# omuses/hqp

Measured on AMD Instinct MI355X. Metric: KKT factor+solve/sec (fp64), higher is better.
Workload: dtype f64; 1 GPU; C4 = BASELINE configs[3], the metric's 10^6-variable DOCP: multistage LQ optimal control QP, K=200 stages, nx=5000 states, nu=50 controls -> n=1015000 me=1005000 m=20000, dense fx/fu handed over as blocks, x_0 fixed, box bounds on u; plugin LQDOCP (STAGED engine), one system per GPU; stages=200, nx=5000, nu=50, n=1015000, me=1005000, m=20000, plugin=LQDOCP, kkt_dim_full=2040000

## Files before the change

### hqp_amd/csrc/staged.hip.h

```cpp
#pragma once
#include <hip/hip_runtime.h>

#include <algorithm>

#include "staged_plan.hpp"
#include "sk_table.hpp"

namespace stg {

using kktdev::double4_t;
using kktdev::mfma_f64;

typedef double double2_t __attribute__((ext_vector_type(2)));

struct StripTab {
  int nranks;
  int cut[17];
  int ld[17];
  long long off[17];
};
struct RectTab {
  int nranks;
  int cut[17];
  struct Block {
    long long off[2];
    int rsplit;
    int pad;
  } blk[16 * 16];
};
static __device__ __forceinline__ int strip_of(const int *cut, int nranks, int j) {
  int p = 0;
  while (p + 1 < nranks && cut[p + 1] <= j) p++;
  return p;
}

struct GemmArgs {
  const double *A;
  long long lda;
  const double *B;
  long long ldb;
  const double *Cin;
  long long ldcin;
  double *C;
  long long ldc;
  int M, N, K;
  double alpha, beta;
  int lower;
  int mirror;
  const int *tile_map;
  const double *zeros;
  const RectTab *rects;
  const StripTab *bstrips;
  unsigned long long *stamps;
};

static const int GEMM_BK = 16;

static inline long long gemm_tiles(int M, int N, int b, int lower) {
  const long long tm = (M + b - 1) / b, tn = (N + b - 1) / b;
  return lower ? tn * (tn + 1) / 2 + (tm > tn ? (tm - tn) * tn : 0) : tm * tn;
}
static inline size_t gemm_lds_bytes(int bm, int bn, int nbuf = 2) { return sizeof(double) * nbuf * GEMM_BK * (size_t)(bm + 16 + bn + 16); }

static inline bool gemm_big_tiles(int M, int N, int lower, int K = 0) {
  const long long t = gemm_tiles(M, N, 128, lower);
  return t >= 384 || (!lower && t >= 160 && t <= 256 && K >= 256 * GEMM_BK);
}

static inline bool gemm_use_split(int M, int N, int K, int lower, int grid);
__device__ __forceinline__ int xcd_swizzle(int bid, int nwg) {
  const int q = nwg >> 3, r = nwg & 7, x = bid & 7;
  return x * q + (x < r ? x : r) + (bid >> 3);
}

template <int BM, int BN, int WGM = 2, int WGN = 2>
struct GemmTile {
  static constexpr int BK = GEMM_BK;
  static constexpr int NW = WGM * WGN, NT = 64 * NW;
  static constexpr int LDA = BM + 16, LDB = BN + 16;
  static constexpr int WM = BM / WGM, WN = BN / WGN, TM = WM / 16, TN = WN / 16;
  static constexpr int LA = BK * BM / 2 / 256, LB = BK * BN / 2 / 256;
  static constexpr int RA = 256 / (BM / 2), RB = 256 / (BN / 2);

  static __device__ __forceinline__ void tile_of(const GemmArgs &g, int t, int &tm, int &tn) {
    if (g.tile_map && BM == 128) {
      const int e = g.tile_map[t];
      tm = e >> 16, tn = e & 0xffff;
    } else if (g.lower) {
      const int tcols = (g.N + BN - 1) / BN, tri = tcols * (tcols + 1) / 2;
      if (t < tri) {
        tm = (int)((sqrtf(8.0f * (float)t + 1.0f) - 1.0f) * 0.5f);
        while ((tm + 1) * (tm + 2) / 2 <= t) tm++;
        while (tm * (tm + 1) / 2 > t) tm--;
        tn = t - tm * (tm + 1) / 2;
      } else {
        tm = tcols + (t - tri) / tcols;
        tn = (t - tri) % tcols;
      }
    } else {
      const int tiles_n = (g.N + BN - 1) / BN, tiles_m = (g.M + BM - 1) / BM;
      constexpr int GM = 8;
      const int grp = t / (GM * tiles_n), first = grp * GM;
      const int rows = min(GM, tiles_m - first);
      const int in = t - grp * GM * tiles_n;
      tm = first + in % rows;
      tn = in / rows;
    }
  }

  static __device__ __forceinline__ void accumulate(const GemmArgs &g, int i0, int j0, int s0, int s1,
                                                    double4_t (&acc)[TM][TN], double *As, double *Bs) {
    static_assert(NT == 256, "the register-staged loop is written for 256 threads");
    const int tid = threadIdx.x, lane = tid & 63, wave = tid >> 6;
    const int wm = wave / WGN, wn = wave % WGN;
    const int lr = lane & 15, lk = lane >> 4;
    const int ca = 2 * (tid % (BM / 2)), ra = tid / (BM / 2);
    const int cb = 2 * (tid % (BN / 2)), rb = tid / (BN / 2);
    const long long acol = (i0 + ca < g.lda) ? i0 + ca : 0;
    const double *Bp = g.B;
    long long ldb = g.ldb;
    int jb = j0;
    if (g.bstrips) {
      const int q = strip_of(g.bstrips->cut, g.bstrips->nranks, j0);
      Bp = g.B + g.bstrips->off[q], ldb = g.bstrips->ld[q], jb = j0 - g.bstrips->cut[q];
    }
    const long long bcol = (jb + cb < ldb) ? jb + cb : 0;
    constexpr int D = (BM * BN <= 64 * 64) ? 4 : 1;
    double2_t sa[D][LA], sb[D][LB];
    const int last = s1 - 1;
    auto gload = [&](double2_t(&xa)[LA], double2_t(&xb)[LB], int slab) {
      const int k0 = (slab < last ? slab : last) * BK;
#pragma unroll
      for (int p = 0; p < LA; p++) {
        const int k = k0 + ra + p * RA, kc = k < g.K ? k : g.K - 1;
        xa[p] = *(const double2_t *)(g.A + (long long)kc * g.lda + acol);
      }
#pragma unroll
      for (int p = 0; p < LB; p++) {
        const int k = k0 + rb + p * RB, kc = k < g.K ? k : g.K - 1;
        xb[p] = *(const double2_t *)(Bp + (long long)kc * ldb + bcol);
      }
    };
    auto lstore = [&](int buf, const double2_t(&xa)[LA], const double2_t(&xb)[LB], int slab) {
      const int k0 = (slab < last ? slab : last) * BK;
#pragma unroll
      for (int p = 0; p < LA; p++) {
        double2_t v = xa[p];
        if (k0 + ra + p * RA >= g.K) v = (double2_t){0.0, 0.0};
        *(double2_t *)(As + (buf * BK + ra + p * RA) * LDA + ca) = v;
      }
#pragma unroll
      for (int p = 0; p < LB; p++) {
        double2_t v = xb[p];
        if (k0 + rb + p * RB >= g.K) v = (double2_t){0.0, 0.0};
        *(double2_t *)(Bs + (buf * BK + rb + p * RB) * LDB + cb) = v;
      }
    };
    auto multiply = [&](int buf) {
      const double *Ab = As + buf * BK * LDA + wm * WM + lr;
      const double *Bb = Bs + buf * BK * LDB + wn * WN + lr;
#pragma unroll
      for (int ks = 0; ks < BK / 4; ks++) {
        double af[TM], bf[TN];
#pragma unroll
        for (int x = 0; x < TM; x++) af[x] = Ab[(ks * 4 + lk) * LDA + 16 * x];
#pragma unroll
        for (int y = 0; y < TN; y++) bf[y] = Bb[(ks * 4 + lk) * LDB + 16 * y];
#pragma unroll
        for (int x = 0; x < TM; x++)
#pragma unroll
          for (int y = 0; y < TN; y++) acc[x][y] = mfma_f64(af[x], bf[y], acc[x][y]);
      }
    };
    if (s1 <= s0) return;
#pragma unroll
    for (int d = 0; d < D; d++) gload(sa[d], sb[d], s0 + d);
    lstore(0, sa[0], sb[0], s0);
    __syncthreads();
    int s = s0;
    for (; s + D <= s1; s += D) {
#pragma unroll
      for (int d = 0; d < D; d++) {
        const int buf = d & 1;
        gload(sa[d], sb[d], s + d + D);
        multiply(D == 1 ? ((s - s0) & 1) : buf);
        lstore(D == 1 ? (((s - s0) & 1) ^ 1) : (buf ^ 1), sa[(d + 1) % D], sb[(d + 1) % D], s + d + 1);
        __syncthreads();
      }
    }
#pragma unroll
    for (int d = 0; d < D - 1; d++) {
      if (s + d < s1) {
        multiply((D == 1 ? (s + d - s0) : d) & 1);
        if (s + d + 1 < s1) lstore(((D == 1 ? (s + d - s0) : d) & 1) ^ 1, sa[(d + 1) % D], sb[(d + 1) % D], s + d + 1);
        __syncthreads();
      }
    }
  }

  static __device__ __forceinline__ void glds16(const double *src, double *lds_row) {
    __builtin_amdgcn_global_load_lds((const __attribute__((address_space(1))) void *)src,
                                     (__attribute__((address_space(3))) void *)lds_row, 16, 0, 0);
  }
  template <bool MASKED>
  static __device__ __forceinline__ void slabs_dma(const GemmArgs &g, const double *pa, const double *pb, const double *zr, int wave,
                                                   int wm, int wn, int lr, int lk, int s0, int s1, unsigned mask,
                                                   double4_t (&acc)[TM][TN], double *As, double *Bs) {
    constexpr int RPW = BK / NW;
    auto dma = [&](int buf, int k0, int p) {
      const int r = wave + NW * (p % RPW), k = k0 + r;
      if (p < RPW)
        glds16(k < g.K ? pa + (long long)k * g.lda : zr, As + (buf * BK + r) * LDA);
      else
        glds16(k < g.K ? pb + (long long)k * g.ldb : zr, Bs + (buf * BK + r) * LDB);
    };
    if (s1 > s0) {
#pragma unroll
      for (int p = 0; p < 2 * RPW; p++) dma(0, s0 * BK, p);
    }
    __syncthreads();
    constexpr int GAP = TM * TN / (2 * RPW);
    for (int s = s0; s < s1; s++) {
      const int buf = (s - s0) & 1;
      const int knext = s + 1 < s1 ? (s + 1) * BK : g.K;
      const double *Ab = As + buf * BK * LDA + wm * WM + lr;
      const double *Bb = Bs + buf * BK * LDB + wn * WN + lr;
#pragma unroll
      for (int ks = 0; ks < BK / 4; ks++) {
        double af[TM], bf[TN];
#pragma unroll
        for (int x = 0; x < TM; x++) af[x] = Ab[(ks * 4 + lk) * LDA + 16 * x];
#pragma unroll
        for (int y = 0; y < TN; y++) bf[y] = Bb[(ks * 4 + lk) * LDB + 16 * y];
#pragma unroll
        for (int x = 0; x < TM; x++)
#pragma unroll
          for (int y = 0; y < TN; y++) {
            if (!MASKED || ((mask >> (x * TN + y)) & 1u)) acc[x][y] = mfma_f64(af[x], bf[y], acc[x][y]);
            if (ks == 0 && (x * TN + y) % GAP == GAP - 1) dma(buf ^ 1, knext, (x * TN + y) / GAP);
          }
      }
      __syncthreads();
    }
  }
  template <bool MASKED>
  static __device__ __forceinline__ void slabs_dma3(const GemmArgs &g, const double *pa, const double *pb, const double *zr, int wave,
                                                    int wm, int wn, int lr, int lk, int s0, int s1, unsigned mask,
                                                    double4_t (&acc)[TM][TN], double *As, double *Bs) {
    constexpr int RPW = BK / NW;
    static_assert(2 * RPW == 4 || 2 * RPW == 8, "the counted waits below are written for 4 or 8 pieces per wave and slab");
    auto dma = [&](int buf, int k0, int p) {
      const int r = wave + NW * (p % RPW), k = k0 + r;
      if (p < RPW)
        glds16(k < g.K ? pa + (long long)k * g.lda : zr, As + (buf * BK + r) * LDA);
      else
        glds16(k < g.K ? pb + (long long)k * g.ldb : zr, Bs + (buf * BK + r) * LDB);
    };
    auto wait_all_but_newest_slab = [&]() {
      if constexpr (2 * RPW == 4)
        asm volatile("s_waitcnt vmcnt(4) lgkmcnt(0)\n\ts_barrier" ::: "memory");
      else
        asm volatile("s_waitcnt vmcnt(8) lgkmcnt(0)\n\ts_barrier" ::: "memory");
    };
#pragma unroll
    for (int p = 0; p < 2 * RPW; p++) dma(0, s1 > s0 ? s0 * BK : g.K, p);
#pragma unroll
    for (int p = 0; p < 2 * RPW; p++) dma(1, s0 + 1 < s1 ? (s0 + 1) * BK : g.K, p);
    wait_all_but_newest_slab();
    constexpr int GAP = TM * TN / (2 * RPW);
    int buf = 0;
    for (int s = s0; s < s1; s++) {
      const int bnext = buf >= 1 ? buf - 1 : 2;
      const int knext = s + 2 < s1 ? (s + 2) * BK : g.K;
      const double *Ab = As + buf * BK * LDA + wm * WM + lr;
      const double *Bb = Bs + buf * BK * LDB + wn * WN + lr;
#pragma unroll
      for (int ks = 0; ks < BK / 4; ks++) {
        double af[TM], bf[TN];
#pragma unroll
        for (int x = 0; x < TM; x++) af[x] = Ab[(ks * 4 + lk) * LDA + 16 * x];
#pragma unroll
        for (int y = 0; y < TN; y++) bf[y] = Bb[(ks * 4 + lk) * LDB + 16 * y];
#pragma unroll
        for (int x = 0; x < TM; x++)
#pragma unroll
          for (int y = 0; y < TN; y++) {
            if (!MASKED || ((mask >> (x * TN + y)) & 1u)) acc[x][y] = mfma_f64(af[x], bf[y], acc[x][y]);
            if (ks == 0 && (x * TN + y) % GAP == GAP - 1) dma(bnext, knext, (x * TN + y) / GAP);
          }
      }
      wait_all_but_newest_slab();
      buf = buf == 2 ? 0 : buf + 1;
    }
    asm volatile("s_waitcnt vmcnt(0)" ::: "memory");
    __syncthreads();
  }
  static __device__ __forceinline__ void accumulate_dma(const GemmArgs &g, int i0, int j0, int s0, int s1,
                                                        double4_t (&acc)[TM][TN], double *As, double *Bs, bool skip_upper = false, int nbuf = 2) {
    static_assert(BM == 128 && BN == 128, "one k-row of a panel must be one 1-KiB wave-instruction");
    static_assert((BK / NW) * NW == BK && TM * TN >= 2 * (BK / NW) && TM * TN <= 32,
                  "pieces are issued behind the multiplications of the first k-step");
    const int tid = threadIdx.x, lane = tid & 63, wave = __builtin_amdgcn_readfirstlane(tid >> 6);
    const int wm = wave / WGN, wn = wave % WGN;
    const int lr = lane & 15, lk = lane >> 4;
    GemmArgs gl = g;
    int jb = j0;
    if (g.bstrips) {
      const int q = strip_of(g.bstrips->cut, g.bstrips->nranks, j0);
      gl.B = g.B + g.bstrips->off[q], gl.ldb = g.bstrips->ld[q], jb = j0 - g.bstrips->cut[q];
    }
    const double *pa = g.A + ((i0 + 2 * lane < g.lda) ? i0 + 2 * lane : 0);
    const double *pb = gl.B + ((jb + 2 * lane < gl.ldb) ? jb + 2 * lane : 0);
    const double *zr = g.zeros + 2 * lane;
    unsigned mask = 0;
#pragma unroll
    for (int x = 0; x < TM; x++)
#pragma unroll
      for (int y = 0; y < TN; y++) {
        const int rb = wm * TM + x, cb = wn * TN + y;
        const bool want = i0 + 16 * rb < g.M && j0 + 16 * cb < g.N && !(skip_upper && cb > rb);
        mask |= (want ? 1u : 0u) << (x * TN + y);
      }
    mask = __builtin_amdgcn_readfirstlane(mask);
    const bool all = mask == (TM * TN == 32 ? 0xffffffffu : (1u << (TM * TN)) - 1u);
    if (nbuf == 3) {
      if (all)
        slabs_dma3<false>(gl, pa, pb, zr, wave, wm, wn, lr, lk, s0, s1, mask, acc, As, Bs);
      else
        slabs_dma3<true>(gl, pa, pb, zr, wave, wm, wn, lr, lk, s0, s1, mask, acc, As, Bs);
    } else if (all)
      slabs_dma<false>(gl, pa, pb, zr, wave, wm, wn, lr, lk, s0, s1, mask, acc, As, Bs);
    else
      slabs_dma<true>(gl, pa, pb, zr, wave, wm, wn, lr, lk, s0, s1, mask, acc, As, Bs);
  }

  static __device__ __forceinline__ void epilogue(const GemmArgs &g, int tm, int tn, const double4_t (&acc)[TM][TN], double *lds) {
    const int tid = threadIdx.x, lane = tid & 63, wave = tid >> 6;
    const int wm = wave / WGN, wn = wave % WGN;
    const int lr = lane & 15, lk = lane >> 4;
    const int i0 = tm * BM, j0 = tn * BN;
    const bool diag = g.lower && tm == tn;
    const double *cin = g.Cin;
    long long ldcin = g.ldcin;
    if (g.rects && g.beta != 0.0) {
      const RectTab &R = *g.rects;
      const int a = strip_of(R.cut, R.nranks, i0), b = strip_of(R.cut, R.nranks, j0);
      const RectTab::Block &blk = R.blk[a * 16 + b];
      const int t = i0 >= blk.rsplit ? 1 : 0, r0 = t ? blk.rsplit : R.cut[a], c0 = R.cut[b];
      ldcin = R.cut[b + 1] - c0;
      cin = g.Cin + blk.off[t] - ((long long)r0 * ldcin + c0);
    }
    constexpr int HC = BN < 64 ? BN : 64, LDT = BM + 2;
    const bool via_lds = g.mirror && !diag && lds != nullptr;
    double4_t val[TM][TN];
#pragma unroll
    for (int x = 0; x < TM; x++)
#pragma unroll
      for (int y = 0; y < TN; y++)
#pragma unroll
        for (int rg = 0; rg < 4; rg++) {
          const int i = i0 + wm * WM + 16 * x + lk + 4 * rg, j = j0 + wn * WN + 16 * y + lr;
          double v = 0.0;
          if (i < g.M && j < g.N && !(diag && i < j)) {
            v = g.alpha * acc[x][y][rg];
            if (g.beta != 0.0) v += g.beta * cin[(long long)i * ldcin + j];
            g.C[(long long)i * g.ldc + j] = v;
            if (g.mirror && i != j && !via_lds) g.C[(long long)j * g.ldc + i] = v;
          }
          val[x][y][rg] = v;
        }
    if (via_lds) {
#pragma unroll
      for (int h = 0; h < BN / HC; h++) {
        if ((wn * WN) / HC == h) {
#pragma unroll
          for (int x = 0; x < TM; x++)
#pragma unroll
            for (int y = 0; y < TN; y++)
#pragma unroll
              for (int rg = 0; rg < 4; rg++)
                lds[(wn * WN - h * HC + 16 * y + lr) * LDT + wm * WM + 16 * x + lk + 4 * rg] = val[x][y][rg];
        }
        __syncthreads();
        for (int jj = wave; jj < HC; jj += NW) {
          const int j = j0 + h * HC + jj;
          if (j >= g.N) break;
          for (int ii = 2 * lane; ii < BM; ii += 128) {
            const int i = i0 + ii;
            double *dst = g.C + (long long)j * g.ldc + i;
            if (i + 1 < g.M && (((size_t)dst) & 15) == 0)
              *(double2_t *)dst = *(const double2_t *)(lds + jj * LDT + ii);
            else {
              if (i < g.M) dst[0] = lds[jj * LDT + ii];
              if (i + 1 < g.M) dst[1] = lds[jj * LDT + ii + 1];
            }
          }
        }
        __syncthreads();
      }
    }
  }
};

constexpr int gemm_waves_per_simd(int nw, int nbuf) { return nbuf == 3 ? nw / 4 : nw / 2; }
template <int BM, int BN, bool DMA = false, int WGM = 2, int WGN = 2, int NBUF = 2>
__global__ void __launch_bounds__(64 * WGM * WGN, gemm_waves_per_simd(WGM * WGN, NBUF)) k_dgemm_tn(GemmArgs g) {
  using T = GemmTile<BM, BN, WGM, WGN>;
  extern __shared__ __attribute__((aligned(16))) double lds[];
  double *As = lds, *Bs = lds + NBUF * T::BK * ((DMA && BM == 64) ? 64 : T::LDA);
  int tm, tn;
  const unsigned long long t0 = g.stamps ? __builtin_amdgcn_s_memrealtime() : 0;
  T::tile_of(g, xcd_swizzle(blockIdx.x, gridDim.x), tm, tn);
  double4_t acc[T::TM][T::TN];
#pragma unroll
  for (int x = 0; x < T::TM; x++)
#pragma unroll
    for (int y = 0; y < T::TN; y++) acc[x][y] = (double4_t){0.0, 0.0, 0.0, 0.0};
  if constexpr (DMA)
    T::accumulate_dma(g, tm * BM, tn * BN, 0, (g.K + T::BK - 1) / T::BK, acc, As, Bs, g.lower && tm == tn, NBUF);
  else
    T::accumulate(g, tm * BM, tn * BN, 0, (g.K + T::BK - 1) / T::BK, acc, As, Bs);
  const unsigned long long t2 = g.stamps ? __builtin_amdgcn_s_memrealtime() : 0;
  T::epilogue(g, tm, tn, acc, lds);
  if (g.stamps && threadIdx.x == 0) {
    asm volatile("s_waitcnt vmcnt(0)" ::: "memory");
    unsigned xcc;
    asm volatile("s_getreg_b32 %0, hwreg(HW_REG_XCC_ID)" : "=s"(xcc));
    g.stamps[4 * blockIdx.x + 0] = t0, g.stamps[4 * blockIdx.x + 1] = (unsigned long long)(xcc & 15);
    g.stamps[4 * blockIdx.x + 2] = t2, g.stamps[4 * blockIdx.x + 3] = __builtin_amdgcn_s_memrealtime();
  }
}

template <int BM, int BN>
__global__ void __launch_bounds__(256) k_dgemm_tn_ks(GemmArgs g, double *__restrict__ part, int nsplit) {
  using T = GemmTile<BM, BN, 2, 2>;
  extern __shared__ __attribute__((aligned(16))) double lds[];
  double *As = lds, *Bs = lds + 2 * T::BK * T::LDA;
  int tm, tn;
  T::tile_of(g, blockIdx.x, tm, tn);
  const int nslab = (g.K + T::BK - 1) / T::BK, L = (nslab + nsplit - 1) / nsplit;
  const int s0 = min(nslab, (int)blockIdx.y * L), s1 = min(nslab, s0 + L);
  double4_t acc[T::TM][T::TN];
#pragma unroll
  for (int x = 0; x < T::TM; x++)
#pragma unroll
    for (int y = 0; y < T::TN; y++) acc[x][y] = (double4_t){0.0, 0.0, 0.0, 0.0};
  T::accumulate(g, tm * BM, tn * BN, s0, s1, acc, As, Bs);
  const int lane = threadIdx.x & 63, wave = threadIdx.x >> 6, wm = wave / 2, wn = wave % 2, lr = lane & 15, lk = lane >> 4;
  double *out = part + (long long)blockIdx.y * g.M * g.N;
#pragma unroll
  for (int x = 0; x < T::TM; x++)
#pragma unroll
    for (int y = 0; y < T::TN; y++)
#pragma unroll
      for (int rg = 0; rg < 4; rg++) {
        const int i = tm * BM + wm * T::WM + 16 * x + lk + 4 * rg, j = tn * BN + wn * T::WN + 16 * y + lr;
        if (i < g.M && j < g.N) out[(long long)i * g.N + j] = acc[x][y][rg];
      }
}
__global__ void k_dgemm_ks_finish(GemmArgs g, const double *__restrict__ part, int nsplit) {
  const long long e = (long long)blockIdx.x * blockDim.x + threadIdx.x, tot = (long long)g.M * g.N;
  if (e >= tot) return;
  double s = 0.0;
  for (int y = 0; y < nsplit; y++) s += part[(long long)y * tot + e];
  const int i = (int)(e / g.N), j = (int)(e % g.N);
  double v = g.alpha * s;
  if (g.beta != 0.0) v += g.beta * g.Cin[(long long)i * g.ldcin + j];
  g.C[(long long)i * g.ldc + j] = v;
}

struct SplitPlan {
  double *ws;
  unsigned *cnt;
  int dp_rounds;
  int whole;
  int nphase;
  int begin[3], count[3], split[3];
  int frac, per, ntiles;
  const SkUnit *table;
  int stride;
};

static inline SplitPlan gemm_split_plan(long long tiles, long long nslab, int grid) {
  SplitPlan sp{};
  const long long smax = std::max<long long>(1, std::min<long long>(16, nslab / 16));
  sp.dp_rounds = (int)(tiles / grid);
  long long R = tiles - (long long)sp.dp_rounds * grid, begin = (long long)sp.dp_rounds * grid;
  sp.whole = (int)begin;
  while (R > 0 && sp.nphase < 2) {
    long long s = std::min<long long>(smax, grid / R), r = R;
    if (s <= 1) {
      s = 1;
      if (sp.nphase == 0 && smax >= 2 && R > grid / 2 && grid % 2 == 0) s = 2, r = grid / 2;
    }
    sp.begin[sp.nphase] = (int)begin, sp.count[sp.nphase] = (int)r, sp.split[sp.nphase] = (int)s;
    sp.nphase++, begin += r, R -= r;
  }
  return sp;
}
static inline SplitPlan gemm_split_plan_frac(long long tiles, long long nslab, int grid) {
  SplitPlan sp{};
  sp.frac = 1, sp.ntiles = (int)tiles;
  sp.per = (int)((tiles * nslab + grid - 1) / grid);
  return sp;
}
static inline long long gemm_split_plan_pieces(const SplitPlan &sp) {
  long long n = 0;
  for (int q = 0; q < sp.nphase; q++) n += (long long)sp.count[q] * sp.split[q];
  return n;
}
static inline long long gemm_split_plan_depth(const SplitPlan &sp, long long nslab) {
  long long d = (long long)sp.dp_rounds * nslab;
  for (int q = 0; q < sp.nphase; q++) d += (nslab + sp.split[q] - 1) / sp.split[q];
  return d;
}
static inline bool gemm_use_split(int M, int N, int K, int lower, int grid) {
  if (grid <= 0 || (long long)M * N < 256LL * 256) return false;
  const long long tiles = gemm_tiles(M, N, 128, lower);
  const long long nslab = (K + GEMM_BK - 1) / GEMM_BK;
  if (nslab < 32) return false;
  if (tiles % grid == 0 || tiles >= 16LL * grid) return false;
  if (tiles > grid * 5 / 8) return true;
  return false;
}
static inline bool gemm_use_frac(int M, int N, int K, int lower, int grid) {
  if (grid <= 0) return false;
  const long long tiles = gemm_tiles(M, N, 128, lower), nslab = (K + GEMM_BK - 1) / GEMM_BK;
  return nslab >= 64 && tiles * 16 >= grid * 5LL && tiles * 8 <= grid * 5LL;
}
template <bool DMA, int WGM = 2, int WGN = 2, int NBUF = 2, int BM = 128, int BN = 128>
__global__ void __launch_bounds__(64 * WGM * WGN, NBUF == 3 ? WGM * WGN / 4 : WGM * WGN / 2) k_dgemm_tn_sk(GemmArgs g, SplitPlan sk) {
  using T = GemmTile<BM, BN, WGM, WGN>;
  extern __shared__ __attribute__((aligned(16))) double lds[];
  double *As = lds, *Bs = lds + NBUF * T::BK * T::LDA;
  unsigned *s_old = (unsigned *)(lds + NBUF * T::BK * (T::LDA + T::LDB));
  const int G = gridDim.x, v = xcd_swizzle(blockIdx.x, G);
  const int nslab = (g.K + T::BK - 1) / T::BK;
  constexpr int SLOT = BM * BN;
  unsigned long long *stamp = g.stamps ? g.stamps + 32 * (long long)blockIdx.x : nullptr;
  if (stamp && threadIdx.x == 0) stamp[0] = __builtin_amdgcn_s_memrealtime();
  if (sk.table) {
    auto unit = [&](const SkUnit u, int r) {
      const int t = u.tile, s0 = u.s0, s1 = u.s1, pieces = u.pieces, j = u.j;
      int tm, tn;
      T::tile_of(g, t, tm, tn);
      double4_t acc[T::TM][T::TN];
#pragma unroll
      for (int x = 0; x < T::TM; x++)
#pragma unroll
        for (int y = 0; y < T::TN; y++) acc[x][y] = (double4_t){0.0, 0.0, 0.0, 0.0};
      if constexpr (DMA)
        T::accumulate_dma(g, tm * BM, tn * BN, s0, s1, acc, As, Bs, g.lower && tm == tn, NBUF);
      else
        T::accumulate(g, tm * BM, tn * BN, s0, s1, acc, As, Bs);
      bool finish = true;
      if (stamp && threadIdx.x == 0 && r < 10) stamp[1 + 3 * r] = __builtin_amdgcn_s_memrealtime();
      if (pieces > 1) {
        double *mine = sk.ws + (long long)(u.slot0 + j) * SLOT;
#pragma unroll
        for (int x = 0; x < T::TM; x++)
#pragma unroll
          for (int y = 0; y < T::TN; y++)
#pragma unroll
            for (int rg = 0; rg < 4; rg++) mine[((x * T::TN + y) * 4 + rg) * T::NT + threadIdx.x] = acc[x][y][rg];
        asm volatile("s_waitcnt vmcnt(0)" ::: "memory");
        __syncthreads();
        if (threadIdx.x == 0) {
          __builtin_amdgcn_fence(__ATOMIC_RELEASE, "agent");
          asm volatile("s_waitcnt vmcnt(0)" ::: "memory");
          *s_old = __hip_atomic_fetch_add(sk.cnt + t, 1u, __ATOMIC_RELAXED, __HIP_MEMORY_SCOPE_AGENT);
        }
        __syncthreads();
        finish = *s_old == (unsigned)(pieces - 1);
        if (finish) {
          if (threadIdx.x == 0) {
            sk.cnt[t] = 0;
            __builtin_amdgcn_fence(__ATOMIC_ACQUIRE, "agent");
            asm volatile("s_waitcnt vmcnt(0)" ::: "memory");
          }
          __syncthreads();
#pragma unroll
          for (int x = 0; x < T::TM; x++)
#pragma unroll
            for (int y = 0; y < T::TN; y++) acc[x][y] = (double4_t){0.0, 0.0, 0.0, 0.0};
          for (int jj = 0; jj < pieces; jj++) {
            const double *theirs = sk.ws + (long long)(u.slot0 + jj) * SLOT;
#pragma unroll
            for (int x = 0; x < T::TM; x++)
#pragma unroll
              for (int y = 0; y < T::TN; y++)
#pragma unroll
                for (int rg = 0; rg < 4; rg++) acc[x][y][rg] += theirs[((x * T::TN + y) * 4 + rg) * T::NT + threadIdx.x];
          }
        }
        __syncthreads();
      }
      if (stamp && threadIdx.x == 0 && r < 10) stamp[2 + 3 * r] = __builtin_amdgcn_s_memrealtime();
      if (finish) T::epilogue(g, tm, tn, acc, lds);
      if (stamp && threadIdx.x == 0 && r < 10) {
        asm volatile("s_waitcnt vmcnt(0)" ::: "memory");
        stamp[3 + 3 * r] = __builtin_amdgcn_s_memrealtime();
      }
      __syncthreads();
    };
    const SkUnit *tab = sk.table + (long long)blockIdx.x * sk.stride;
    for (int r = 0; r < sk.stride; r++) {
      const SkUnit u = tab[r];
      if (u.tile < 0) break;
      unit(u, r);
    }
    return;
  }
  if (sk.frac) {
    const int U = sk.ntiles * nslab, per = sk.per;
    const int lo = min(U, v * per), hi = min(U, lo + per), t_first = lo / nslab;
    for (int x = lo; x < hi;) {
      const int t = x / nslab, s0 = x - t * nslab, s1 = min(nslab, s0 + (hi - x));
      const int w_first = (t * nslab) / per, w_last = ((t + 1) * nslab - 1) / per, pieces = w_last - w_first + 1;
      int tm, tn;
      T::tile_of(g, t, tm, tn);
      double4_t acc[T::TM][T::TN];
#pragma unroll
      for (int xx = 0; xx < T::TM; xx++)
#pragma unroll
        for (int y = 0; y < T::TN; y++) acc[xx][y] = (double4_t){0.0, 0.0, 0.0, 0.0};
      if constexpr (DMA)
        T::accumulate_dma(g, tm * BM, tn * BN, s0, s1, acc, As, Bs, g.lower && tm == tn, NBUF);
      else
        T::accumulate(g, tm * BM, tn * BN, s0, s1, acc, As, Bs);
      bool finish = true;
      if (pieces > 1) {
        double *mine = sk.ws + (long long)(2 * v + (t == t_first ? 0 : 1)) * SLOT;
#pragma unroll
        for (int xx = 0; xx < T::TM; xx++)
#pragma unroll
          for (int y = 0; y < T::TN; y++)
#pragma unroll
            for (int rg = 0; rg < 4; rg++) mine[((xx * T::TN + y) * 4 + rg) * T::NT + threadIdx.x] = acc[xx][y][rg];
        asm volatile("s_waitcnt vmcnt(0)" ::: "memory");
        __syncthreads();
        if (threadIdx.x == 0) {
          __builtin_amdgcn_fence(__ATOMIC_RELEASE, "agent");
          asm volatile("s_waitcnt vmcnt(0)" ::: "memory");
          *s_old = __hip_atomic_fetch_add(sk.cnt + t, 1u, __ATOMIC_RELAXED, __HIP_MEMORY_SCOPE_AGENT);
        }
        __syncthreads();
        finish = *s_old == (unsigned)(pieces - 1);
        if (finish) {
          if (threadIdx.x == 0) {
            sk.cnt[t] = 0;
            __builtin_amdgcn_fence(__ATOMIC_ACQUIRE, "agent");
            asm volatile("s_waitcnt vmcnt(0)" ::: "memory");
          }
          __syncthreads();
#pragma unroll
          for (int xx = 0; xx < T::TM; xx++)
#pragma unroll
            for (int y = 0; y < T::TN; y++) acc[xx][y] = (double4_t){0.0, 0.0, 0.0, 0.0};
          for (int w = w_first; w <= w_last; w++) {
            const double *theirs = sk.ws + (long long)(2 * w + (t == (w * per) / nslab ? 0 : 1)) * SLOT;
#pragma unroll
            for (int xx = 0; xx < T::TM; xx++)
#pragma unroll
              for (int y = 0; y < T::TN; y++)
#pragma unroll
                for (int rg = 0; rg < 4; rg++) acc[xx][y][rg] += theirs[((xx * T::TN + y) * 4 + rg) * T::NT + threadIdx.x];
          }
        }
        __syncthreads();
      }
      if (finish) T::epilogue(g, tm, tn, acc, lds);
      __syncthreads();
      x += s1 - s0;
    }
    return;
  }
  const int n_whole = sk.whole;
  int n_units = n_whole;
  for (int q = 0; q < sk.nphase; q++) n_units += sk.count[q] * sk.split[q];
  int r = 0;
  for (int u = v; u < n_units; r++) {
    int q = -1;
    int t = u, s0 = 0, s1 = nslab, cnt = G, pieces = 1, ti = 0, pbase = 0;
    if (u >= n_whole) {
      int rel = u - n_whole;
      q = 0;
      while (q + 1 < sk.nphase && rel >= sk.count[q] * sk.split[q]) rel -= sk.count[q] * sk.split[q], pbase += sk.count[q] * sk.split[q], q++;
      cnt = sk.count[q], pieces = sk.split[q];
      ti = rel % cnt;
      const int L = (nslab + pieces - 1) / pieces, j = rel / cnt;
      t = sk.begin[q] + ti, s0 = min(nslab, j * L), s1 = min(nslab, s0 + L);
    }
    const int u_now = u;
    {
      int nu = n_units;
      if (u + G < n_whole)
        nu = u + G;
      else {
        int base = n_whole, qq = 0;
        if (u >= n_whole) base += pbase + cnt * pieces, qq = q + 1;
        for (; qq < sk.nphase && nu == n_units; qq++) {
          if (v < sk.count[qq] * sk.split[qq]) nu = base + v;
          base += sk.count[qq] * sk.split[qq];
        }
      }
      if (threadIdx.x == 0) s_old[1] = (unsigned)nu;
    }
    int tm, tn;
    T::tile_of(g, t, tm, tn);
    double4_t acc[T::TM][T::TN];
#pragma unroll
    for (int x = 0; x < T::TM; x++)
#pragma unroll
      for (int y = 0; y < T::TN; y++) acc[x][y] = (double4_t){0.0, 0.0, 0.0, 0.0};
    if constexpr (DMA)
      T::accumulate_dma(g, tm * BM, tn * BN, s0, s1, acc, As, Bs, g.lower && tm == tn, NBUF);
    else
      T::accumulate(g, tm * BM, tn * BN, s0, s1, acc, As, Bs);
    bool finish = true;
    if (stamp && threadIdx.x == 0 && r < 5) stamp[1 + 3 * r] = __builtin_amdgcn_s_memrealtime();
    if (pieces > 1) {
      double *mine = sk.ws + (long long)(u_now - n_whole) * SLOT;
#pragma unroll
      for (int x = 0; x < T::TM; x++)
#pragma unroll
        for (int y = 0; y < T::TN; y++)
#pragma unroll
          for (int rg = 0; rg < 4; rg++) mine[((x * T::TN + y) * 4 + rg) * T::NT + threadIdx.x] = acc[x][y][rg];
      asm volatile("s_waitcnt vmcnt(0)" ::: "memory");
      __syncthreads();
      if (threadIdx.x == 0) {
        __builtin_amdgcn_fence(__ATOMIC_RELEASE, "agent");
        asm volatile("s_waitcnt vmcnt(0)" ::: "memory");
        *s_old = __hip_atomic_fetch_add(sk.cnt + t, 1u, __ATOMIC_RELAXED, __HIP_MEMORY_SCOPE_AGENT);
      }
      __syncthreads();
      finish = *s_old == (unsigned)(pieces - 1);
      if (finish) {
        if (threadIdx.x == 0) {
          sk.cnt[t] = 0;
          __builtin_amdgcn_fence(__ATOMIC_ACQUIRE, "agent");
          asm volatile("s_waitcnt vmcnt(0)" ::: "memory");
        }
        __syncthreads();
#pragma unroll
        for (int x = 0; x < T::TM; x++)
#pragma unroll
          for (int y = 0; y < T::TN; y++) acc[x][y] = (double4_t){0.0, 0.0, 0.0, 0.0};
        for (int jj = 0; jj < pieces; jj++) {
          const double *theirs = sk.ws + (long long)(pbase + jj * cnt + ti) * SLOT;
#pragma unroll
          for (int x = 0; x < T::TM; x++)
#pragma unroll
            for (int y = 0; y < T::TN; y++)
#pragma unroll
              for (int rg = 0; rg < 4; rg++) acc[x][y][rg] += theirs[((x * T::TN + y) * 4 + rg) * T::NT + threadIdx.x];
        }
      }
      __syncthreads();
    }
    if (stamp && threadIdx.x == 0 && r < 5) stamp[2 + 3 * r] = __builtin_amdgcn_s_memrealtime();
    if (finish) T::epilogue(g, tm, tn, acc, lds);
    if (stamp && threadIdx.x == 0 && r < 5) {
      asm volatile("s_waitcnt vmcnt(0)" ::: "memory");
      stamp[3 + 3 * r] = __builtin_amdgcn_s_memrealtime();
    }
    __syncthreads();
    u = (int)s_old[1];
    __syncthreads();
  }
}
static inline size_t gemm_sk_lds_bytes(int nbuf = 2) { return gemm_lds_bytes(128, 128, nbuf) + 16; }

enum { GEMM_REG4 = 0, GEMM_DMA4 = 1, GEMM_DMA8 = 2, GEMM_DMA8X3 = 3 };
static inline int gemm_wgs_per_cu(int variant) { return variant == GEMM_DMA8X3 ? 1 : 2; }
static inline void gemm_launch_plain(int variant, unsigned tiles, hipStream_t s, const GemmArgs &g, int cus = 0) {
  if (variant == GEMM_DMA8 && cus > 0 && (int)tiles <= cus) variant = GEMM_DMA8X3;
  if (variant == GEMM_DMA8X3)
    k_dgemm_tn<128, 128, true, 2, 4, 3><<<tiles, 512, gemm_lds_bytes(128, 128, 3), s>>>(g);
  else if (variant == GEMM_DMA8)
    k_dgemm_tn<128, 128, true, 2, 4><<<tiles, 512, gemm_lds_bytes(128, 128), s>>>(g);
  else if (variant == GEMM_DMA4)
    k_dgemm_tn<128, 128, true><<<tiles, 256, gemm_lds_bytes(128, 128), s>>>(g);
  else
    k_dgemm_tn<128, 128><<<tiles, 256, gemm_lds_bytes(128, 128), s>>>(g);
}
static inline void gemm_launch_split(int variant, int grid, hipStream_t s, const GemmArgs &g, const SplitPlan &sk) {
  if (variant == GEMM_DMA8X3)
    k_dgemm_tn_sk<true, 2, 4, 3><<<grid, 512, gemm_sk_lds_bytes(3), s>>>(g, sk);
  else if (variant == GEMM_DMA8)
    k_dgemm_tn_sk<true, 2, 4><<<grid, 512, gemm_sk_lds_bytes(), s>>>(g, sk);
  else if (variant == GEMM_DMA4)
    k_dgemm_tn_sk<true><<<grid, 256, gemm_sk_lds_bytes(), s>>>(g, sk);
  else
    k_dgemm_tn_sk<false><<<grid, 256, gemm_sk_lds_bytes(), s>>>(g, sk);
}
static inline bool gemm_tiles_6432(int M, int N, int K, int lower, int mirror, int cus) {
  return cus > 0 && !lower && !mirror && gemm_tiles(M, N, 64, 0) <= 2LL * cus && K >= 16 * GEMM_BK;
}
static inline hipError_t gemm_set_attributes() {
  hipError_t e = hipSuccess;
  auto set = [&](const void *f, size_t bytes) {
    const hipError_t r = hipFuncSetAttribute(f, hipFuncAttributeMaxDynamicSharedMemorySize, (int)bytes);
    if (e == hipSuccess) e = r;
  };
  set((const void *)k_dgemm_tn<128, 128>, gemm_lds_bytes(128, 128));
  set((const void *)k_dgemm_tn<128, 128, true>, gemm_lds_bytes(128, 128));
  set((const void *)k_dgemm_tn<128, 128, true, 2, 4>, gemm_lds_bytes(128, 128));
  set((const void *)k_dgemm_tn<64, 64>, gemm_lds_bytes(64, 64));
  set((const void *)k_dgemm_tn<64, 32>, gemm_lds_bytes(64, 32));
  set((const void *)k_dgemm_tn_ks<64, 64>, gemm_lds_bytes(64, 64));
  set((const void *)k_dgemm_tn_sk<false>, gemm_sk_lds_bytes());
  set((const void *)k_dgemm_tn_sk<true>, gemm_sk_lds_bytes());
  set((const void *)k_dgemm_tn_sk<true, 2, 4>, gemm_sk_lds_bytes());
  set((const void *)k_dgemm_tn<128, 128, true, 2, 4, 3>, gemm_lds_bytes(128, 128, 3));
  set((const void *)k_dgemm_tn_sk<true, 2, 4, 3>, gemm_sk_lds_bytes(3));
  return e;
}
static inline bool gemm_sk_table_from_env() {
  const char *r = getenv("HQPKKT_SK_TABLE");
  return !r || atoi(r) != 0;
}
static inline int gemm_variant_from_env() {
  if (getenv("HQPKKT_NO_LDSDMA")) return GEMM_REG4;
  const char *w = getenv("HQPKKT_DGEMM_WAVES");
  if (w && atoi(w) == 4) return GEMM_DMA4;
  return GEMM_DMA8;
}

struct HTerm {
  int s1, s2, wi;
};
__global__ void k_st_add_h(int nent, const long long *__restrict__ dst, const int *__restrict__ tptr,
                           const HTerm *__restrict__ terms, const double *__restrict__ vals,
                           const double *__restrict__ wt, double *__restrict__ G, int add) {
  const int e = blockIdx.x * blockDim.x + threadIdx.x;
  if (e >= nent) return;
  double s = 0.0;
  for (int k = tptr[e]; k < tptr[e + 1]; k++) s += vals[terms[k].s1] * vals[terms[k].s2] * wt[terms[k].wi];
  if (add)
    G[dst[e]] += s;
  else
    G[dst[e]] = s;
}

__global__ void k_st_add_h_owned(int nent, const long long *__restrict__ dst, const int *__restrict__ tptr,
                                 const HTerm *__restrict__ terms, const double *__restrict__ vals,
                                 const double *__restrict__ wt, double *__restrict__ G, long long ld,
                                 const unsigned *__restrict__ owned, int ntc) {
  const int e = blockIdx.x * blockDim.x + threadIdx.x;
  if (e >= nent) return;
  const long long d = dst[e];
  const int t = (int)(d / ld >> 7) * ntc + (int)(d % ld >> 7);
  if (!((owned[t >> 5] >> (t & 31)) & 1u)) return;
  double s = 0.0;
  for (int k = tptr[e]; k < tptr[e + 1]; k++) s += vals[terms[k].s1] * vals[terms[k].s2] * wt[terms[k].wi];
  G[d] += s;
}

__global__ void k_st_scatter(long long nent, const long long *__restrict__ dst, const double *__restrict__ vals,
                             double *__restrict__ F, double *__restrict__ misc) {
  const long long e = (long long)blockIdx.x * blockDim.x + threadIdx.x;
  if (e >= nent) return;
  const long long d = dst[e];
  if (d >= 0)
    F[d] = vals[e];
  else if (d <= -2)
    misc[-(d + 2)] = vals[e];
}
__global__ void k_st_check(int nchk, const int *__restrict__ idx, const int *__restrict__ kind,
                           const double *__restrict__ vals, int *__restrict__ status) {
  const int e = blockIdx.x * blockDim.x + threadIdx.x;
  if (e >= nchk) return;
  const double v = vals[idx[e]];
  if (kind[e] == 0 ? v != -1.0 : v == 0.0) atomicExch(status, 6);
}

struct ArgMax {
  double v;
  int i;
};
__device__ __forceinline__ ArgMax better(ArgMax a, ArgMax b) { return (b.v > a.v || (b.v == a.v && b.i < a.i)) ? b : a; }
__device__ __forceinline__ ArgMax block_argmax(ArgMax a, ArgMax *red) {
  const double vmax = kktdev::wave_max_dpp(a.v);
  const unsigned long long hit = __ballot(a.v == vmax);
  const int src = hit ? __ffsll((long long)hit) - 1 : 0;
  a.v = vmax;
  a.i = __builtin_amdgcn_readlane(a.i, src);
  __syncthreads();
  if ((threadIdx.x & 63) == 0) red[threadIdx.x >> 6] = a;
  __syncthreads();
  ArgMax r = red[0];
  for (int w = 1; w < (int)(blockDim.x >> 6); w++)
    if (red[w].v > r.v) r = red[w];
  return r;
}

#ifdef HQPKKT_STAMPS
__device__ int g_gj_stamps[32];
#define GSTAMP(slot)                                                                              \
  do {                                                                                            \
    if (threadIdx.x == 0 && s == 10) g_gj_stamps[slot] = (int)__builtin_amdgcn_s_memtime();       \
  } while (0)
#else
#define GSTAMP(slot)
#endif
#ifndef HQPKKT_GJ_RB
#define HQPKKT_GJ_RB 2
#endif
template <int RB = 1>
__device__ int gj_inverse(double *a, int q, int ld, int *ip, int *ir, int *ic, double *colv, double *rowv,
                          ArgMax *red) {
  const int tid = threadIdx.x, nt = blockDim.x;
  const int ty = tid >> 4, tx = tid & 15, RS = nt >> 4;
  const double INF = __longlong_as_double(0x7ff0000000000000LL);
  const long long ABS = 0x7fffffffffffffffLL, INFB = 0x7ff0000000000000LL;
  for (int j = tid; j < q; j += nt) ip[j] = 0;
  __syncthreads();
  int bad = 0;
  long long bb = -1;
  int bi = 0x7fffffff;
  for (int r = ty; r < q; r += RS)
    for (int c = tx; c < q; c += 16) {
      const long long bits = __double_as_longlong(a[r * ld + c]) & ABS;
      if (bits > bb) bb = bits, bi = r * q + c;
    }
  for (int s = 0; s < q; s++) {
    GSTAMP(0);
    ArgMax best = block_argmax(ArgMax{bb < 0 ? -1.0 : (bb > INFB ? INF : __longlong_as_double(bb)), bi}, red);
    GSTAMP(1);
    const int irow = best.i / q, icol = best.i - irow * q;
    if (!(best.v > 0.0) || best.v == INF) bad = 1;
    if (irow != icol)
      for (int c = tid; c < q; c += nt) {
        const double x = a[irow * ld + c];
        a[irow * ld + c] = a[icol * ld + c];
        a[icol * ld + c] = x;
      }
    if (tid == 0) ip[icol] = 1, ir[s] = irow, ic[s] = icol;
    __syncthreads();
    GSTAMP(2);
    const double pinv = bad ? 1.0 : 1.0 / a[icol * ld + icol];
    for (int c = tid; c < q; c += nt) {
      colv[c] = (c == icol) ? 0.0 : a[c * ld + icol];
      rowv[c] = (c == icol ? 1.0 : a[icol * ld + c]) * pinv;
    }
    __syncthreads();
    for (int c = tid; c < q; c += nt) {
      if (c != icol) a[c * ld + icol] = 0.0;
      a[icol * ld + c] = rowv[c];
    }
    __syncthreads();
    GSTAMP(3);
    bb = -1, bi = 0x7fffffff;
    for (int c0 = tx; c0 < q; c0 += 128) {
      double rv[8];
      int cc[8];
      bool cfree[8];
#pragma unroll
      for (int u = 0; u < 8; u++) {
        const int c = c0 + 16 * u;
        cc[u] = c < q ? c : q - 1;
        rv[u] = rowv[cc[u]];
        cfree[u] = c < q && ip[cc[u]] == 0;
      }
      for (int r0 = ty; r0 < q; r0 += RS * RB) {
        double x[RB][8];
#pragma unroll
        for (int k = 0; k < RB; k++) {
          const int r = min(r0 + k * RS, q - 1);
#pragma unroll
          for (int u = 0; u < 8; u++) x[k][u] = a[r * ld + cc[u]];
        }
#pragma unroll
        for (int k = 0; k < RB; k++) {
          const int r = r0 + k * RS, rr = min(r, q - 1);
          const double cr = colv[rr];
          const bool rfree = r < q && ip[rr] == 0;
#pragma unroll
          for (int u = 0; u < 8; u++) {
            const int c = c0 + 16 * u;
            const double v = fma(-rv[u], cr, x[k][u]);
            if (r < q && c < q) a[r * ld + c] = v;
            const long long bits = __double_as_longlong(v) & ABS;
            if (rfree && cfree[u] && bits > bb) bb = bits, bi = r * q + c;
          }
        }
      }
    }
    GSTAMP(4);
  }
  __syncthreads();
  for (int s = q - 1; s >= 0; s--) {
    const int r1 = ir[s], c1 = ic[s];
    if (r1 != c1)
      for (int r = tid; r < q; r += nt) {
        const double x = a[r * ld + r1];
        a[r * ld + r1] = a[r * ld + c1];
        a[r * ld + c1] = x;
      }
    __syncthreads();
  }
  return bad;
}

template <int NB>
__device__ int gj_inverse_reg(double *a, int q, int ld, int *ip, int *pc_of_row, double *colv, double *rowv, ArgMax *red) {
  const int tid = threadIdx.x, ty = tid >> 4, tx = tid & 15;
  const double INF = __longlong_as_double(0x7ff0000000000000LL);
  double m[NB][2 * NB];
  int rfree = 0, cfree = 0;
#pragma unroll
  for (int i = 0; i < NB; i++) {
    const int r = ty + 16 * i;
    if (r < q) rfree |= 1 << i;
    if (tx + 16 * i < q) cfree |= 1 << i;
#pragma unroll
    for (int j = 0; j < NB; j++) {
      const int c = tx + 16 * j;
      m[i][j] = (r < q && c < q) ? a[r * ld + c] : 0.0;
      m[i][NB + j] = (r == c && r < q) ? 1.0 : 0.0;
    }
  }
  __syncthreads();
  int bad = 0;
  for (int s = 0; s < q; s++) {
    ArgMax best{-1.0, 0x7fffffff};
#pragma unroll
    for (int i = 0; i < NB; i++)
#pragma unroll
      for (int j = 0; j < NB; j++)
        if ((rfree >> i & 1) && (cfree >> j & 1)) {
          const double v = fabs(m[i][j]);
          best = better(best, ArgMax{v == v ? v : INF, (ty + 16 * i) * q + tx + 16 * j});
        }
    best = block_argmax(best, red);
    const int pr = best.i / q, pc = best.i - pr * q;
    if (!(best.v > 0.0) || best.v == INF) bad = 1;
    if ((pr & 15) == ty) {
      const int i = pr >> 4;
#pragma unroll
      for (int ii = 0; ii < NB; ii++)
        if (ii == i) {
#pragma unroll
          for (int j = 0; j < 2 * NB; j++) rowv[tx + 16 * j] = m[ii][j];
        }
    }
    if ((pc & 15) == tx) {
      const int j = pc >> 4;
#pragma unroll
      for (int jj = 0; jj < NB; jj++)
        if (jj == j) {
#pragma unroll
          for (int i = 0; i < NB; i++) colv[ty + 16 * i] = m[i][jj];
        }
    }
    if (tid == 0) pc_of_row[pr] = pc;
    __syncthreads();
    const double piv = rowv[(pc & 15) + 16 * (pc >> 4)];
    const double pinv = bad ? 1.0 : 1.0 / piv;
    double rv[2 * NB];
#pragma unroll
    for (int j = 0; j < 2 * NB; j++) rv[j] = rowv[tx + 16 * j] * pinv;
#pragma unroll
    for (int i = 0; i < NB; i++) {
      const int r = ty + 16 * i;
      const double f = colv[r];
      if (r == pr) {
#pragma unroll
        for (int j = 0; j < 2 * NB; j++) m[i][j] = rv[j];
      } else {
#pragma unroll
        for (int j = 0; j < 2 * NB; j++) m[i][j] -= f * rv[j];
      }
    }
    if ((pr & 15) == ty) rfree &= ~(1 << (pr >> 4));
    if ((pc & 15) == tx) cfree &= ~(1 << (pc >> 4));
    __syncthreads();
  }
#pragma unroll
  for (int i = 0; i < NB; i++) {
    const int r = ty + 16 * i;
    if (r < q) {
      const int dst = pc_of_row[r];
#pragma unroll
      for (int j = 0; j < NB; j++) {
        const int c = tx + 16 * j;
        if (c < q) a[dst * ld + c] = m[i][NB + j];
      }
    }
  }
  __syncthreads();
  (void)ip;
  return bad;
}
template <int NB>
__device__ int gj_inverse_reg_spd(double *a, int q, int ld, double *colv, double *rowv) {
  const int tid = threadIdx.x, ty = tid >> 4, tx = tid & 15;
  double m[NB][NB];
#pragma unroll
  for (int i = 0; i < NB; i++) {
    const int r = ty + 16 * i;
#pragma unroll
    for (int j = 0; j < NB; j++) {
      const int c = tx + 16 * j;
      m[i][j] = (r < q && c < q) ? a[r * ld + c] : (r == c ? 1.0 : 0.0);
    }
  }
  __syncthreads();
  int bad = 0;
  for (int s = 0; s < q; s++) {
    if ((s & 15) == ty) {
      const int i = s >> 4;
#pragma unroll
      for (int ii = 0; ii < NB; ii++)
        if (ii == i) {
#pragma unroll
// ... 1634 lines not shown
```

Baseline: 0.8205 KKT factor+solve/s.

## Add register-prefetched k-step pipeline for table-driven split-K DGEMM kernel

Adds a new slab loop for the two-buffer LDS-DMA GEMM that double-buffers MFMA fragments in registers. It loads the next k-step's fragments from LDS while the current k-step's MFMAs issue, and uses sched_group_barrier to interleave LDS reads with MFMAs. A dedicated table-only specialization of the split-K kernel is instantiated and launched when the SK table is present, which drops the non-table code paths from that kernel. The aim is to hide LDS read latency and cut register pressure or branching in the stream-K GEMM. The cost is extra fragment registers and tighter manual scheduling that could hurt occupancy.

```diff
diff --git a/hqp_amd/csrc/staged.hip.h b/hqp_amd/csrc/staged.hip.h
--- a/hqp_amd/csrc/staged.hip.h
+++ b/hqp_amd/csrc/staged.hip.h
@@ -81,6 +81,7 @@
   static constexpr int WM = BM / WGM, WN = BN / WGN, TM = WM / 16, TN = WN / 16;
   static constexpr int LA = BK * BM / 2 / 256, LB = BK * BN / 2 / 256;
   static constexpr int RA = 256 / (BM / 2), RB = 256 / (BN / 2);
+  static constexpr int NBUF_PF = 0;
 
   static __device__ __forceinline__ void tile_of(const GemmArgs &g, int t, int &tm, int &tn) {
     if (g.tile_map && BM == 128) {
@@ -295,6 +296,85 @@
     asm volatile("s_waitcnt vmcnt(0)" ::: "memory");
     __syncthreads();
   }
+  template <bool MASKED>
+  static __device__ __forceinline__ void slabs_dma_pf(const GemmArgs &g, const double *pa, const double *pb, const double *zr, int wave,
+                                                      int wm, int wn, int lr, int lk, int s0, int s1, unsigned mask,
+                                                      double4_t (&acc)[TM][TN], double *As, double *Bs) {
+    constexpr int RPW = BK / NW;
+    auto dma = [&](int buf, int k0, int p) {
+      const int r = wave + NW * (p % RPW), k = k0 + r, kc = k < g.K ? k : g.K - 1;
+      const double *src = p < RPW ? pa + (long long)kc * g.lda : pb + (long long)kc * g.ldb;
+      glds16(k < g.K ? src : zr, p < RPW ? As + (buf * BK + r) * LDA : Bs + (buf * BK + r) * LDB);
+    };
+    struct Frag {
+      double a[TM], b[TN];
+    };
+    const double *Aw = As + wm * WM + lr + lk * LDA, *Bw = Bs + wn * WN + lr + lk * LDB;
+    auto load = [&](Frag &f, int buf, int ks) {
+#pragma unroll
+      for (int x = 0; x < TM; x++) f.a[x] = Aw[(buf * BK + ks * 4) * LDA + 16 * x];
+#pragma unroll
+      for (int y = 0; y < TN; y++) f.b[y] = Bw[(buf * BK + ks * 4) * LDB + 16 * y];
+    };
+    auto mma = [&](const Frag &f) {
+#pragma unroll
+      for (int x = 0; x < TM; x++)
+#pragma unroll
+        for (int y = 0; y < TN; y++)
+          if (!MASKED || ((mask >> (x * TN + y)) & 1u)) acc[x][y] = mfma_f64(f.a[x], f.b[y], acc[x][y]);
+    };
+    auto wait_lds = [] {
+      __builtin_amdgcn_sched_barrier(0);
+      __builtin_amdgcn_s_waitcnt(0xC07F);
+      __builtin_amdgcn_sched_barrier(0);
+    };
+    auto pin = [](bool reads) {
+      if constexpr (!MASKED) {
+        if (reads) __builtin_amdgcn_sched_group_barrier(0x100, (TM + TN) / 2, 0);
+        __builtin_amdgcn_sched_group_barrier(0x008, TM * TN, 0);
+      }
+    };
+    constexpr int GAP = TM * TN / (2 * RPW);
+    static_assert(BK / 4 == 4 && TM % 2 == 0 && TN % 2 == 0, "four k-steps per slab, fragments read in pairs");
+    if (s1 <= s0) {
+      __syncthreads();
+      return;
+    }
+#pragma unroll
+    for (int p = 0; p < 2 * RPW; p++) dma(0, s0 * BK, p);
+    __syncthreads();
+    Frag f0, f1;
+    auto slab = [&](int s, bool more) {
+      const int buf = (s - s0) & 1;
+      const int knext = more ? (s + 1) * BK : g.K;
+      load(f1, buf, 1);
+      __builtin_amdgcn_sched_barrier(0);
+#pragma unroll
+      for (int x = 0; x < TM; x++)
+#pragma unroll
+        for (int y = 0; y < TN; y++) {
+          if (!MASKED || ((mask >> (x * TN + y)) & 1u)) acc[x][y] = mfma_f64(f0.a[x], f0.b[y], acc[x][y]);
+          if ((x * TN + y) % GAP == GAP - 1) dma(buf ^ 1, knext, (x * TN + y) / GAP);
+        }
+      wait_lds();
+      load(f0, buf, 2);
+      mma(f1);
+      pin(true);
+      wait_lds();
+      load(f1, buf, 3);
+      mma(f0);
+      pin(true);
+      __builtin_amdgcn_sched_barrier(0);
+      __syncthreads();
+      if (more) load(f0, buf ^ 1, 0);
+      mma(f1);
+      pin(more);
+    };
+    load(f0, 0, 0);
+    int s = s0;
+    for (; s + 1 < s1; s++) slab(s, true);
+    slab(s, false);
+  }
   static __device__ __forceinline__ void accumulate_dma(const GemmArgs &g, int i0, int j0, int s0, int s1,
                                                         double4_t (&acc)[TM][TN], double *As, double *Bs, bool skip_upper = false, int nbuf = 2) {
     static_assert(BM == 128 && BN == 128, "one k-row of a panel must be one 1-KiB wave-instruction");
@@ -323,7 +403,12 @@
       }
     mask = __builtin_amdgcn_readfirstlane(mask);
     const bool all = mask == (TM * TN == 32 ? 0xffffffffu : (1u << (TM * TN)) - 1u);
-    if (nbuf == 3) {
+    if (nbuf == NBUF_PF) {
+      if (all)
+        slabs_dma_pf<false>(gl, pa, pb, zr, wave, wm, wn, lr, lk, s0, s1, mask, acc, As, Bs);
+      else
+        slabs_dma_pf<true>(gl, pa, pb, zr, wave, wm, wn, lr, lk, s0, s1, mask, acc, As, Bs);
+    } else if (nbuf == 3) {
       if (all)
         slabs_dma3<false>(gl, pa, pb, zr, wave, wm, wn, lr, lk, s0, s1, mask, acc, As, Bs);
       else
@@ -528,8 +613,9 @@
   const long long tiles = gemm_tiles(M, N, 128, lower), nslab = (K + GEMM_BK - 1) / GEMM_BK;
   return nslab >= 64 && tiles * 16 >= grid * 5LL && tiles * 8 <= grid * 5LL;
 }
-template <bool DMA, int WGM = 2, int WGN = 2, int NBUF = 2, int BM = 128, int BN = 128>
+template <bool DMA, int WGM = 2, int WGN = 2, int NBUF = 2, int BM = 128, int BN = 128, bool TABLE = false>
 __global__ void __launch_bounds__(64 * WGM * WGN, NBUF == 3 ? WGM * WGN / 4 : WGM * WGN / 2) k_dgemm_tn_sk(GemmArgs g, SplitPlan sk) {
+  static_assert(!TABLE || (DMA && NBUF == 2), "the table kernel is the two-buffer LDS-DMA form");
   using T = GemmTile<BM, BN, WGM, WGN>;
   extern __shared__ __attribute__((aligned(16))) double lds[];
   double *As = lds, *Bs = lds + NBUF * T::BK * T::LDA;
@@ -539,7 +625,7 @@
   constexpr int SLOT = BM * BN;
   unsigned long long *stamp = g.stamps ? g.stamps + 32 * (long long)blockIdx.x : nullptr;
   if (stamp && threadIdx.x == 0) stamp[0] = __builtin_amdgcn_s_memrealtime();
-  if (sk.table) {
+  if (TABLE || sk.table) {
     auto unit = [&](const SkUnit u, int r) {
       const int t = u.tile, s0 = u.s0, s1 = u.s1, pieces = u.pieces, j = u.j;
       int tm, tn;
@@ -549,7 +635,9 @@
       for (int x = 0; x < T::TM; x++)
 #pragma unroll
         for (int y = 0; y < T::TN; y++) acc[x][y] = (double4_t){0.0, 0.0, 0.0, 0.0};
-      if constexpr (DMA)
+      if constexpr (TABLE)
+        T::accumulate_dma(g, tm * BM, tn * BN, s0, s1, acc, As, Bs, g.lower && tm == tn, T::NBUF_PF);
+      else if constexpr (DMA)
         T::accumulate_dma(g, tm * BM, tn * BN, s0, s1, acc, As, Bs, g.lower && tm == tn, NBUF);
       else
         T::accumulate(g, tm * BM, tn * BN, s0, s1, acc, As, Bs);
@@ -611,6 +699,7 @@
     }
     return;
   }
+  if constexpr (TABLE) return;
   if (sk.frac) {
     const int U = sk.ntiles * nslab, per = sk.per;
     const int lo = min(U, v * per), hi = min(U, lo + per), t_first = lo / nslab;
@@ -788,6 +877,8 @@
 static inline void gemm_launch_split(int variant, int grid, hipStream_t s, const GemmArgs &g, const SplitPlan &sk) {
   if (variant == GEMM_DMA8X3)
     k_dgemm_tn_sk<true, 2, 4, 3><<<grid, 512, gemm_sk_lds_bytes(3), s>>>(g, sk);
+  else if (variant == GEMM_DMA8 && sk.table)
+    k_dgemm_tn_sk<true, 2, 4, 2, 128, 128, true><<<grid, 512, gemm_sk_lds_bytes(), s>>>(g, sk);
   else if (variant == GEMM_DMA8)
     k_dgemm_tn_sk<true, 2, 4><<<grid, 512, gemm_sk_lds_bytes(), s>>>(g, sk);
   else if (variant == GEMM_DMA4)
@@ -813,6 +904,7 @@
   set((const void *)k_dgemm_tn_sk<false>, gemm_sk_lds_bytes());
   set((const void *)k_dgemm_tn_sk<true>, gemm_sk_lds_bytes());
   set((const void *)k_dgemm_tn_sk<true, 2, 4>, gemm_sk_lds_bytes());
+  set((const void *)k_dgemm_tn_sk<true, 2, 4, 2, 128, 128, true>, gemm_sk_lds_bytes());
   set((const void *)k_dgemm_tn<128, 128, true, 2, 4, 3>, gemm_lds_bytes(128, 128, 3));
   set((const void *)k_dgemm_tn_sk<true, 2, 4, 3>, gemm_sk_lds_bytes(3));
   return e;
```

Measured after the change: 0.8203 KKT factor+solve/s (median of 4 runs). About the same (-0.0%).
